# CESNET/GPUJPEG

Hardware: AMD Instinct MI355X
Metric: Mpix/s encode+decode (8K RGB q75) (higher is better)
Workload: dtype f32

## Files before the change

### gpujpeg_amd/csrc/gj_enc_assemble.hip

```cpp
#include "gj_enc_internal.h"

#define GJ_GATHER_PRELOAD 8
#define GJ_GATHER_MARK_DW 2048
__global__ __launch_bounds__(256) void k_gather(const GjTail T0)
{
    GjTail T = T0;
    {
        const size_t fz = blockIdx.z;
        T.piece += fz * T0.f_tail; T.group += fz * T0.f_tail; T.group_other += fz * T0.f_tail;
        T.temp += fz * T0.f_temp; T.seg_bytes += fz * T0.f_seg; T.seg_ff += fz * T0.f_seg;
        T.jpeg += fz * T0.f_jpeg; T.d_result += fz * 2;
        if (T.h_result) T.h_result += fz * 2;
    }
    __shared__ uint32_t s_tmp[4];
    __shared__ __attribute__((aligned(16))) uint8_t s_mark[4][GJ_GATHER_MARK_DW];
    const int i = threadIdx.x, lane = i & 63, wave = i >> 6;
    const uint32_t P = T.npieces, NG = T.ngroups;
    const uint32_t p0 = blockIdx.x * 4u, p = p0 + (uint32_t)wave;
    const bool have = p < P;
    if (blockIdx.x == 0)
        for (uint32_t g = i; g < NG; g += 256) T.group_other[g] = 0;
    const uint32_t scan = gj_tail_scan_of(T, have ? p : 0u);
    const uint32_t t = (have ? p : 0u) - gj_pick4(T.scan_first, scan), seg0 = t * T.spt, scan_segs = gj_pick4(T.segs, scan);
    const uint32_t nseg = have ? min(T.spt, scan_segs - seg0) : 0u;
    const uint32_t s0 = gj_pick4(T.seg_first, scan) + seg0;
    const uint64_t src_block = (uint64_t)gj_pick4(T.block_first, scan) + (uint64_t)seg0 * T.seg_blocks;
    const uint32_t* const src = reinterpret_cast<const uint32_t*>(T.temp + src_block * GJ_TEMP_BYTES_PER_BLOCK);
    const uint64_t room = T.temp_blocks > src_block ? T.temp_blocks - src_block : 0u;
    const uint32_t src_dw = (uint32_t)min((uint64_t)nseg * T.seg_blocks, room) * (GJ_TEMP_BYTES_PER_BLOCK / 4u);
    const uint32_t ga = p0 >> 5;
    uint32_t before = 0, all = 0;
    for (uint32_t g0 = 0; g0 < NG; g0 += 1024) {
        uint32_t v[4];
#pragma unroll
        for (int u = 0; u < 4; u++) {
            const uint32_t g = g0 + (uint32_t)u * 256u + (uint32_t)i;
            v[u] = g < NG ? T.group[g] : 0u;
        }
#pragma unroll
        for (int u = 0; u < 4; u++) {
            const uint32_t g = g0 + (uint32_t)u * 256u + (uint32_t)i;
            all += v[u];
            before += g < ga ? v[u] : 0u;
        }
    }
    if ((uint32_t)i < (p0 & 31u)) before += T.piece[(ga << 5) + i];
    uint32_t in_front = 0;
    if (wave > 0 && have) in_front += T.piece[p0];
    if (wave > 1 && have) in_front += T.piece[p0 + 1];
    if (wave > 2 && have) in_front += T.piece[p0 + 2];
    uint32_t nb = 0, ff = 0;
    if ((uint32_t)lane < nseg) {
        nb = T.seg_bytes[s0 + lane];
        ff = T.seg_ff[s0 + lane];
    }
    uint32_t pre[GJ_GATHER_PRELOAD];
#pragma unroll
    for (int m = 0; m < GJ_GATHER_PRELOAD; m++) {
        const uint32_t d = (uint32_t)m * 64u + (uint32_t)lane;
        pre[m] = d < src_dw ? src[d] : 0u;
    }
    uint32_t done_bytes, all_bytes;
    gj_wg256_incl_scan(before, s_tmp, &done_bytes);
    gj_wg256_incl_scan(all, s_tmp, &all_bytes);
    const uint64_t total = (uint64_t)T.main_hdr + gj_pick4(T.hdr_end, gj_tail_scan_of(T, P - 1)) + all_bytes + 2u;
    const bool overflow = total > T.capacity;
    if (p0 + 4 >= P && i == 0) {
        T.d_result[0] = (uint32_t)total;
        T.d_result[1] = overflow ? 1u : 0u;
        if (T.h_result) {
            T.h_result[0] = (uint32_t)total;
            T.h_result[1] = overflow ? 1u : 0u;
        }
    }
    if (!have || overflow) return;
    const uint32_t F = T.main_hdr + gj_pick4(T.hdr_end, scan) + done_bytes + in_front;
    uint8_t* const out = T.jpeg;
    if (t == 0) {
        const uint32_t h1 = gj_pick4(T.hdr_end, scan), h0 = scan == 0 ? 0u : gj_pick4(T.hdr_end, scan - 1);
        for (uint32_t b = lane; b < h1 - h0; b += 64) out[F - (h1 - h0) + b] = T.scan_hdr[h0 + b];
    }
    const uint32_t last = scan_segs - seg0 - 1u;
    const uint32_t ndw = (nb + 3u) >> 2, olen = nb + ff + ((uint32_t)lane < nseg && (uint32_t)lane != last ? 2u : 0u);
    const uint32_t dwi = gj_wave_incl_scan(ndw), dwb = dwi - ndw;
    const uint32_t oi = gj_wave_incl_scan(olen), ob = F + oi - olen;
    const uint32_t ffi = gj_wave_incl_scan(ff);
    const uint32_t total_dw = (uint32_t)__builtin_amdgcn_readlane((int)dwi, 63);
    const uint32_t end = F + (uint32_t)__builtin_amdgcn_readlane((int)oi, 63);
    if (p == P - 1 && lane == 0) {
        out[end] = 0xFF;
        out[end + 1] = 0xD9;
    }
    const uint32_t seg_a = ob - 4u * dwb - (ffi - ff);
    const uint32_t seg_e = (dwi - 1u) | ((nb - 4u * (ndw - 1u)) << 28);
    uint8_t* const mark = s_mark[wave];
    uint32_t ffrun = 0, segs_before = 0;
    for (uint32_t c0 = 0; c0 < total_dw; c0 += GJ_GATHER_MARK_DW) {
        const uint32_t c1 = min(total_dw, c0 + (uint32_t)GJ_GATHER_MARK_DW);
        gj_wave_sync();
#pragma unroll
        for (int z = 0; z < GJ_GATHER_MARK_DW / 256; z++) reinterpret_cast<uint32_t*>(mark)[z * 64 + lane] = 0;
        gj_wave_sync();
        if ((uint32_t)lane < nseg && dwb >= c0 && dwb < c1) mark[dwb - c0] = 1;
        gj_wave_sync();
        for (uint32_t m = c0 >> 6; m * 64u < c1; m++) {
            const uint32_t d = m * 64u + (uint32_t)lane;
            const bool live = d < total_dw;
            uint32_t v = 0;
            if (m < GJ_GATHER_PRELOAD) {
#pragma unroll
                for (int q = 0; q < GJ_GATHER_PRELOAD; q++)
                    if (m == (uint32_t)q) v = pre[q];
            } else if (live) {
                v = src[d];
            }
            const uint32_t seg = gj_wave_incl_scan(live ? mark[d - c0] : 0u) + segs_before - 1u;
            const int sidx = (int)((live ? seg : 0u) << 2);
            const uint32_t a = (uint32_t)__builtin_amdgcn_ds_bpermute(sidx, (int)seg_a), e = (uint32_t)__builtin_amdgcn_ds_bpermute(sidx, (int)seg_e);
            const bool ends = live && d == (e & 0x0FFFFFFFu);
            const int vb = live ? (ends ? (int)(e >> 28) : 4) : 0;
            const uint32_t ffm = live ? ((v & 0x7F7F7F7Fu) + 0x01010101u) & v & 0x80808080u : 0u;
            const uint32_t ffc = (uint32_t)__builtin_popcount(ffm);
            const uint32_t fi = gj_wave_incl_scan(ffc) + ffrun;
            if (live) {
                uint32_t q = a + 4u * d + (fi - ffc);
                if (ffc == 0 && vb == 4) {
                    *reinterpret_cast<gj_u32_unaligned*>(out + q) = v;
                    q += 4;
                } else {
#pragma unroll
                    for (int b = 0; b < 4; b++)
                        if (b < vb) {
                            const uint32_t byte = (v >> (8 * b)) & 0xFFu;
                            out[q++] = (uint8_t)byte;
                            if (byte == 0xFFu) out[q++] = 0;
                        }
                }
                if (ends && seg != last) {
                    out[q] = 0xFF;
                    out[q + 1] = (uint8_t)(0xD0 + ((seg0 + seg) & 7u));
                }
            }
            ffrun = (uint32_t)__builtin_amdgcn_readlane((int)fi, 63);
            segs_before = (uint32_t)__builtin_amdgcn_readlane((int)seg, 63) + 1u;
        }
    }
}

__device__ __forceinline__ uint32_t gj_segment_out_size(const gj_enc_job& J, int s, uint32_t* hdr)
{
    const GjSeg sg = gj_segment(J.g, s);
    *hdr = 0;
    if (sg.first_in_scan) {
        const int scan = J.g.interleaved ? 0 : sg.comp;
        *hdr = J.scan_hdr_offset[scan + 1] - J.scan_hdr_offset[scan];
    }
    return J.d_seg_bytes[s] + J.d_seg_ff[s] + (sg.last_in_scan ? 0u : 2u);
}

__device__ __forceinline__ uint32_t gj_wg1024_incl_scan(uint32_t v, uint32_t* s_w, uint32_t* total)
{
    const int lane = threadIdx.x & 63, wave = threadIdx.x >> 6;
    const uint32_t inc = gj_wave_incl_scan(v);
    __syncthreads();
    if (lane == 63) s_w[wave] = inc;
    __syncthreads();
    uint32_t off = 0, all = 0;
#pragma unroll
    for (int w = 0; w < 16; w++) {
        const uint32_t x = s_w[w];
        if (w < wave) off += x;
        all += x;
    }
    if (total) *total = all;
    return inc + off;
}

__global__ __launch_bounds__(1024) void k_scan_segments(const gj_enc_job J, unsigned long long* __restrict__ partial, const uint32_t epoch)
{
    __shared__ uint32_t s_w[16];
    const int S = J.g.segment_count;
    const int s = blockIdx.x * 1024 + threadIdx.x;
    uint32_t hdr = 0, v = 0;
    if (s < S) v = gj_segment_out_size(J, s, &hdr);
    uint32_t total;
    const uint32_t inc = gj_wg1024_incl_scan(v + hdr, s_w, &total);
    if (threadIdx.x == 0)
        __hip_atomic_store(&partial[blockIdx.x], ((unsigned long long)epoch << 32) | total, __ATOMIC_RELEASE, __HIP_MEMORY_SCOPE_AGENT);
    uint32_t pre = 0;
    for (unsigned t = threadIdx.x; t < blockIdx.x; t += 1024) {
        unsigned long long p;
        do {
            p = __hip_atomic_load(&partial[t], __ATOMIC_ACQUIRE, __HIP_MEMORY_SCOPE_AGENT);
        } while ((uint32_t)(p >> 32) != epoch);
        pre += (uint32_t)p;
    }
    uint32_t base;
    gj_wg1024_incl_scan(pre, s_w, &base);
    base += J.main_hdr_size;
    if (s < S) J.d_seg_out[s] = base + inc - v;
    if (s == S - 1) {
        const uint32_t end = base + inc;
        const uint32_t size = end + 2;
        J.d_seg_out[S] = end;
        J.d_result[0] = size;
        J.d_result[1] = (uint64_t)size > J.jpeg_capacity ? 1u : 0u;
        if (J.h_result) {
            J.h_result[0] = size;
            J.h_result[1] = (uint64_t)size > J.jpeg_capacity ? 1u : 0u;
        }
    }
}

__global__ __launch_bounds__(256) void k_assemble(const gj_enc_job J)
{
    const gj_geom& g = J.g;
    const int s0 = (blockIdx.x * 4 + (threadIdx.x >> 6)) * GJ_ASM_SEGS;
    const int lane = threadIdx.x & 63;
    if (s0 >= g.segment_count || J.d_result[1]) return;
    uint8_t* out = J.d_jpeg;
    uint32_t raw4[GJ_ASM_SEGS], o4[GJ_ASM_SEGS], w4[GJ_ASM_SEGS];
    const uint8_t* src4[GJ_ASM_SEGS];
#pragma unroll
    for (int q = 0; q < GJ_ASM_SEGS; q++) {
        const int s = min(s0 + q, g.segment_count - 1);
        raw4[q] = s0 + q < g.segment_count ? J.d_seg_bytes[s] : 0u;
        o4[q] = J.d_seg_out[s];
        src4[q] = J.d_temp + gj_segment(g, s).first_block * GJ_TEMP_BYTES_PER_BLOCK;
    }
#pragma unroll
    for (int q = 0; q < GJ_ASM_SEGS; q++) w4[q] = (uint32_t)lane * 4u < raw4[q] ? *reinterpret_cast<const uint32_t*>(src4[q] + lane * 4) : 0u;
#pragma unroll
    for (int q = 0; q < GJ_ASM_SEGS; q++) {
        const int s = s0 + q;
        if (s >= g.segment_count) break;
        const GjSeg sg = gj_segment(g, s);
        const uint32_t raw = raw4[q];
        const uint8_t* src = src4[q];
        uint32_t o = o4[q];
        if (sg.first_in_scan) {
            const int scan = g.interleaved ? 0 : sg.comp;
            const uint32_t h0 = J.scan_hdr_offset[scan], hn = J.scan_hdr_offset[scan + 1] - h0;
            for (uint32_t b = lane; b < hn; b += 64) out[o - hn + b] = J.d_scan_hdr[h0 + b];
        }
        for (uint32_t c0 = 0; c0 < raw; c0 += 256) {
            const uint32_t idx = c0 + lane * 4;
            uint32_t w = w4[q];
            int vb = 0;
            if (idx < raw) {
                if (c0) w = *reinterpret_cast<const uint32_t*>(src + idx);
                vb = (int)min(4u, raw - idx);
            }
            int cnt = vb;
#pragma unroll
            for (int b = 0; b < 4; b++)
                if (b < vb && ((w >> (8 * b)) & 0xFFu) == 0xFFu) cnt++;
            const uint32_t inc = gj_wave_incl_scan((uint32_t)cnt);
            uint32_t p = o + inc - (uint32_t)cnt;
#pragma unroll
            for (int b = 0; b < 4; b++) {
                if (b < vb) {
                    const uint32_t byte = (w >> (8 * b)) & 0xFFu;
                    out[p++] = (uint8_t)byte;
                    if (byte == 0xFFu) out[p++] = 0;
                }
            }
            o += (uint32_t)__builtin_amdgcn_readlane((int)inc, 63);
        }
        if (lane == 0) {
            if (!sg.last_in_scan) {
                out[o] = 0xFF;
                out[o + 1] = (uint8_t)(0xD0 + (sg.index_in_scan & 7));
            }
            if (s == g.segment_count - 1) {
                out[o] = 0xFF;
                out[o + 1] = 0xD9;
            }
        }
    }
}

#define GJ_MAX_HEADER_SIZE (65536 - 100)
__global__ __launch_bounds__(256) void k_segment_info(const gj_enc_job J)
{
    const gj_geom& g = J.g;
    const int s = blockIdx.x * 256 + threadIdx.x;
    if (s >= g.segment_count || J.d_result[1]) return;
    const GjSeg sg = gj_segment(g, s);
    const int scan = g.interleaved ? 0 : sg.comp;
    const int first = g.interleaved ? 0 : g.comp[scan].first_segment;
    const int segs = g.interleaved ? g.segment_count : g.comp[scan].segment_count;
    const uint32_t data0 = J.d_seg_out[first];
    const uint32_t hdr_begin = data0 - (J.scan_hdr_offset[scan + 1] - J.scan_hdr_offset[scan]);
    for (int e = sg.index_in_scan; e <= (sg.last_in_scan ? segs : sg.index_in_scan); e++) {
        uint32_t pos;
        if (e < segs) pos = J.d_seg_out[first + e] - data0;
        else pos = J.d_seg_out[first + segs - 1] + J.d_seg_bytes[first + segs - 1] + J.d_seg_ff[first + segs - 1] - data0;
        const uint32_t byte = (uint32_t)e * 4u;
        const uint32_t chunk = byte / GJ_MAX_HEADER_SIZE, within = byte % GJ_MAX_HEADER_SIZE;
        uint8_t* p = J.d_jpeg + hdr_begin + J.scan_info_payload[scan] + chunk * (GJ_MAX_HEADER_SIZE + 5u) + within;
        p[0] = (uint8_t)(pos >> 24); p[1] = (uint8_t)(pos >> 16); p[2] = (uint8_t)(pos >> 8); p[3] = (uint8_t)pos;
    }
}
```

### gpujpeg_amd/csrc/gj_encode.hip

```cpp
#include "gj_enc_internal.h"

static GjTail gj_make_tail(const gj_enc_job* job, const unsigned pieces, const unsigned (&scan_first)[GJ_MAX_COMP], const unsigned spt)
{
    const gj_geom& g = job->g;
    GjTail T;
    for (int s = 0; s < GJ_MAX_COMP; s++) {
        T.scan_first[s] = scan_first[s];
        T.hdr_end[s] = job->scan_hdr_offset[s + 1];
        const bool own_scan = !g.interleaved && s < g.comp_count;
        T.seg_first[s] = own_scan ? (uint32_t)g.comp[s].first_segment : 0u;
        T.segs[s] = own_scan ? (uint32_t)g.comp[s].segment_count : (uint32_t)g.segment_count;
        T.block_first[s] = own_scan ? (uint32_t)(g.comp[s].data_offset / 64) : 0u;
    }
    T.spt = spt;
    T.seg_blocks = (uint32_t)g.seg_blocks;
    const unsigned ngcap = GJ_TAIL_GROUPS_CAP(g.segment_count);
    T.group = job->d_tail + (job->tail_set & 1) * ngcap;
    T.group_other = job->d_tail + ((job->tail_set + 1) & 1) * ngcap;
    T.ngroups = (pieces + 31) / 32;
    T.piece = job->d_tail + 2 * ngcap;
    T.npieces = pieces;
    T.temp = job->d_temp;
    T.temp_blocks = (uint64_t)g.block_count;
    T.seg_bytes = job->d_seg_bytes;
    T.seg_ff = job->d_seg_ff;
    T.jpeg = job->d_jpeg;
    T.capacity = job->jpeg_capacity;
    T.scan_hdr = job->d_scan_hdr;
    T.main_hdr = job->main_hdr_size;
    T.d_result = job->d_result;
    T.h_result = job->h_result;
    const bool batch = job->batch.count > 1;
    T.f_raw = batch ? job->batch.raw : 0;
    T.f_temp = batch ? job->batch.temp : 0;
    T.f_jpeg = batch ? job->batch.jpeg : 0;
    T.f_seg = batch ? job->batch.seg : 0;
    T.f_tail = batch ? job->batch.tail : 0;
    return T;
}


static int gj_blocks_kernel_mode(const gj_geom& g)
{
    if (g.no_transform) return 1;
    if (g.pixel_format != GJ_PF_444_P012 || g.comp_count != 3) return -1;
    const int from = g.color_space, to = g.color_space_internal;
    const bool none = from == to || from == GJ_CS_NONE || to == GJ_CS_NONE;
    if (!none && !(from == GJ_CS_RGB && (to == GJ_CS_BT601 || to == GJ_CS_BT601_256 || to == GJ_CS_BT709))) return -1;
    return 0;
}

static bool gj_is_uyvy_layout(const gj_enc_job* job)
{
    const gj_geom& g = job->g;
    return job->use_fused && g.pixel_format == GJ_PF_422_P1020 && g.comp_count == 3 && g.no_transform == 0 &&
           (g.color_space == g.color_space_internal || g.color_space == GJ_CS_NONE || g.color_space_internal == GJ_CS_NONE) &&
           g.comp[0].samp_h == 2 && g.comp[0].samp_v == 1 && g.comp[1].samp_h == 1 && g.comp[1].samp_v == 1 && g.comp[2].samp_h == 1 &&
           g.comp[2].samp_v == 1 && g.comp[0].blocks_x == 2 * g.comp[1].blocks_x && g.comp[0].blocks_y == g.comp[1].blocks_y &&
           g.comp[2].blocks_x == g.comp[1].blocks_x && g.comp[2].blocks_y == g.comp[1].blocks_y;
}
static int gj_tile_kernel(const gj_enc_job* job)
{
    const gj_geom& g = job->g;
    if (job->stage != GJ_ENC_STAGE_ALL) return 0;
    const bool segs_ok = g.restart_interval > 0 && g.seg_blocks <= 256 && g.seg_blocks >= 256 / GJ_ENC_MAX_SPT;
    gj_encode_kernel_t whole = (job->use_fused && !job->keep_coefs) ? gj_encode_kernel(g) : nullptr;
    if (whole && job->tune.enc_by_blocks > 0 && gj_blocks_kernel_mode(g) == 0) whole = nullptr;
    if (gj_is_uyvy_layout(job) && !job->keep_coefs && g.interleaved && segs_ok && g.blocks_per_mcu == 4 && g.mcu_count == g.comp[1].blocks_x * g.comp[1].blocks_y &&
        g.comp[1].type == g.comp[2].type && !job->tune.enc_no_whole422)
        return 1;
    if (!whole && job->use_fused && !job->keep_coefs && segs_ok && gj_blocks_kernel_mode(g) >= 0) return 2;
    return whole ? 3 : 0;
}

extern "C" int gj_hip_encode_batchable(const gj_enc_job* job)
{
    return job->use_fused && !job->keep_coefs && !job->channel_remap && !job->flipped && !job->segment_info && gj_tile_kernel(job) != 0;
}

extern "C" int gj_hip_encode_tiles(const gj_enc_job* job) { return gj_tile_kernel(job) != 0; }

extern "C" int gj_hip_encode(const gj_enc_job* job, gj_stream_t stream, gj_event_t ev[GJ_ENC_EVENTS])
{
    hipStream_t st = (hipStream_t)stream;
    const gj_geom& g = job->g;
    if (g.blocks_per_mcu > GJ_MAX_MCU_BLOCKS) return -1;
    const unsigned frames = job->batch.count > 1 ? job->batch.count : 1u;
    if (frames > 1 && (!gj_hip_encode_batchable(job) || frames > 65535u)) return -1;
    if (job->stage != GJ_ENC_STAGE_ALL && (frames > 1 || (job->stage == GJ_ENC_STAGE_COUNT && !job->d_huff_freq))) return -1;
    gj_hip_note_reset();
    const bool code_only = job->stage == GJ_ENC_STAGE_CODE;
    if (ev && !code_only) GJ_HIP_CHECK(hipEventRecord((hipEvent_t)ev[0], st));
    if (job->channel_remap && !code_only) {
        const unsigned n = (unsigned)g.width * (unsigned)g.height;
        hipLaunchKernelGGL(k_channel_remap, dim3((n + 255) / 256), dim3(256), 0, st, g, const_cast<uint8_t*>(job->d_raw), job->channel_remap & 0xFFFFu);
    }
    bool tiles = true;
    GjTail T;
    T.npieces = 0;
    const int tile_kernel = gj_tile_kernel(job);
    gj_encode_kernel_t whole = tile_kernel == 3 ? gj_encode_kernel(g) : nullptr;
    gj_fused_kernel_t fused = job->use_fused ? gj_fused_kernel(g) : nullptr;
    const bool uyvy = gj_is_uyvy_layout(job);
    if (tile_kernel == 1) {
        if (ev) GJ_HIP_CHECK(hipEventRecord((hipEvent_t)ev[1], st));
        if (ev) GJ_HIP_CHECK(hipEventRecord((hipEvent_t)ev[2], st));
        const int spt = 256 / g.seg_blocks;
        const unsigned wgs = ((unsigned)g.segment_count + spt - 1) / spt;
        T = gj_make_tail(job, wgs, {0u, ~0u, ~0u, ~0u}, (unsigned)spt);
        hipLaunchKernelGGL(gj_encode_uyvy422_kernel(), dim3(wgs, 1, frames), dim3(256), 0, st, g, job->d_raw, job->d_fwd_q[0], job->d_fwd_q[1], job->d_huff_lut,
                           job->d_temp, job->d_seg_bytes, job->d_seg_ff, T);
    } else if (tile_kernel == 2) {
        if (ev) GJ_HIP_CHECK(hipEventRecord((hipEvent_t)ev[1], st));
        if (ev) GJ_HIP_CHECK(hipEventRecord((hipEvent_t)ev[2], st));
        const int spt = 256 / g.seg_blocks;
        unsigned wgs = 0, scan_first[GJ_MAX_COMP] = {0u, ~0u, ~0u, ~0u};
        if (g.interleaved) wgs = ((unsigned)g.segment_count + spt - 1) / spt;
        else
            for (int c = 0; c < g.comp_count; c++) {
                scan_first[c] = wgs;
                wgs += ((unsigned)g.comp[c].segment_count + spt - 1) / spt;
            }
        T = gj_make_tail(job, wgs, scan_first, (unsigned)spt);
        hipLaunchKernelGGL(gj_encode_blocks_kernel(gj_blocks_kernel_mode(g) != 0), dim3(wgs, 1, frames), dim3(256), 0, st, g, job->d_raw, job->d_fwd_q[0],
                           job->d_fwd_q[1], job->d_huff_lut, job->d_temp, job->d_seg_bytes, job->d_seg_ff, T);
    } else if (whole) {
        if (ev) GJ_HIP_CHECK(hipEventRecord((hipEvent_t)ev[1], st));
        if (ev) GJ_HIP_CHECK(hipEventRecord((hipEvent_t)ev[2], st));
        const int spt = 256 / g.seg_blocks;
        const unsigned wgs = ((unsigned)g.comp[0].segment_count + spt - 1) / spt;
        T = gj_make_tail(job, 3 * wgs, {0u, wgs, 2 * wgs, ~0u}, (unsigned)spt);
        const unsigned split_up_to = job->tune.enc_split >= 0 ? (unsigned)job->tune.enc_split : (unsigned)gj_hip_cu_count() * 4u / 3u;
        const bool split = wgs * frames <= split_up_to;
        if (split) whole = gj_encode_kernel(g, true);
        unsigned grid_x = wgs;
        const unsigned tail = job->tune.enc_tail >= 0 ? (unsigned)job->tune.enc_tail : 32u;
        T.tail_from = 0xFFFFFFFFu;
        T.tiles = wgs;
        if (!split && frames == 1 && tail > 0 && wgs > tail && (job->tune.enc_tail > 0 || wgs > (unsigned)gj_hip_cu_count() * 4u)) {
            T.tail_from = wgs - tail;
            grid_x = wgs + 2u * tail;
        }
        hipLaunchKernelGGL(whole, dim3(grid_x, split ? 3 : 1, frames), dim3(256), 0, st, g, job->d_raw, job->d_fwd_q[0], job->d_fwd_q[1], job->d_huff_lut, job->d_temp,
                           job->d_seg_bytes, job->d_seg_ff, T);
    } else {
    tiles = false;
    if (code_only) {
    } else if (uyvy) {
        if (ev) GJ_HIP_CHECK(hipEventRecord((hipEvent_t)ev[1], st));
        const unsigned nm = (unsigned)(g.comp[1].blocks_x * g.comp[1].blocks_y);
        hipLaunchKernelGGL(gj_fused_uyvy422_kernel(), dim3((nm + 255) / 256), dim3(256), 0, st, g, job->d_raw, job->d_coefs, job->d_fwd_q[0], job->d_fwd_q[1]);
    } else if (fused) {
        if (ev) GJ_HIP_CHECK(hipEventRecord((hipEvent_t)ev[1], st));
        const unsigned nb = (unsigned)(g.comp[0].blocks_x * g.comp[0].blocks_y);
        hipLaunchKernelGGL(fused, dim3((nb + 255) / 256), dim3(256), 0, st, g, job->d_raw, job->d_coefs, job->d_fwd_q[0],
                           job->d_fwd_q[1]);
    } else {
        if (g.no_transform) {
            hipLaunchKernelGGL(k_copy_planes_in, dim3(2048), dim3(256), 0, st, g, job->d_raw, job->d_planes);
        } else {
            const unsigned n = (unsigned)g.raw_width * (unsigned)g.height;
            hipLaunchKernelGGL(k_preprocess, dim3((n + 255) / 256), dim3(256), 0, st, g, job->d_raw, job->d_planes);
        }
        if (job->flipped) hipLaunchKernelGGL(k_flip_planes, dim3(1024), dim3(256), 0, st, g, job->d_planes);
        if (ev) GJ_HIP_CHECK(hipEventRecord((hipEvent_t)ev[1], st));
        hipLaunchKernelGGL(k_dct, dim3(((unsigned)g.block_count + 255) / 256), dim3(256), 0, st, g, job->d_planes, job->d_coefs,
                           job->d_fwd_q[0], job->d_fwd_q[1]);
    }
    if (job->stage == GJ_ENC_STAGE_COUNT) {
        if (ev) GJ_HIP_CHECK(hipEventRecord((hipEvent_t)ev[6], st));
        GJ_HIP_CHECK(hipMemsetAsync(job->d_huff_freq, 0, 1024 * sizeof(uint32_t), st));
        const unsigned total = (unsigned)g.segment_count * (unsigned)g.seg_blocks;
        const unsigned fill = (unsigned)gj_hip_cu_count() * 4u, wgs = (total + 255) / 256 < fill ? (total + 255) / 256 : fill;
        hipLaunchKernelGGL(k_huffman_count, dim3(wgs), dim3(256), 0, st, g, job->d_coefs, job->d_huff_freq);
        if (ev) GJ_HIP_CHECK(hipEventRecord((hipEvent_t)ev[7], st));
        return (hipGetLastError() == hipSuccess && !gj_hip_noted()) ? 0 : -1;
    }
    if (ev) GJ_HIP_CHECK(hipEventRecord((hipEvent_t)ev[2], st));
    const int B = g.seg_blocks;
    const int spt = B <= 256 ? 256 / B : 1;
    const unsigned tiles = ((unsigned)g.segment_count + spt - 1) / spt;
    hipLaunchKernelGGL(k_huffman, dim3(tiles), dim3(256), 0, st, g, job->d_coefs, job->d_huff_lut, job->d_temp, job->d_seg_bytes,
                       job->d_seg_ff);
    }
    if (ev) GJ_HIP_CHECK(hipEventRecord((hipEvent_t)ev[3], st));
    if (tiles)
        hipLaunchKernelGGL(k_gather, dim3((T.npieces + 3) / 4, 1, frames), dim3(256), 0, st, T);
    const bool seg_info = job->segment_info && g.restart_interval > 0;
    const unsigned scan_wgs = ((unsigned)g.segment_count + 1023) / 1024;
    if (!tiles || seg_info)
        hipLaunchKernelGGL(k_scan_segments, dim3(scan_wgs), dim3(1024), 0, st, *job, (unsigned long long*)job->d_scan_partial, job->epoch);
    if (ev) GJ_HIP_CHECK(hipEventRecord((hipEvent_t)ev[4], st));
    if (!tiles)
        hipLaunchKernelGGL(k_assemble, dim3(((unsigned)g.segment_count + 4 * GJ_ASM_SEGS - 1) / (4 * GJ_ASM_SEGS)), dim3(256), 0, st, *job);
    if (seg_info)
        hipLaunchKernelGGL(k_segment_info, dim3(((unsigned)g.segment_count + 255) / 256), dim3(256), 0, st, *job);
    if (ev) GJ_HIP_CHECK(hipEventRecord((hipEvent_t)ev[5], st));
    return (hipGetLastError() == hipSuccess && !gj_hip_noted()) ? 0 : -1;
}
```

Measured before the change: 179,200.

## Vectorize gather to four dwords per lane and use wave-local prefix sums

The gather kernel now has each lane process four consecutive dwords through uint4 loads. Segment indices come from a packed 4-byte mark word, FF counts are summed per lane before one wave scan, and the common no-FF, non-ending dwords take a fast store path. The workgroup-wide scans over group sums are replaced by per-wave scans, so each wave reads all groups itself and no LDS barrier is needed. This cuts scan and bpermute overhead per byte moved, but adds redundant per-wave group reads and assumes 16-byte alignment of the source.

```diff
diff --git a/gpujpeg_amd/csrc/gj_enc_assemble.hip b/gpujpeg_amd/csrc/gj_enc_assemble.hip
--- a/gpujpeg_amd/csrc/gj_enc_assemble.hip
+++ b/gpujpeg_amd/csrc/gj_enc_assemble.hip
@@ -1,6 +1,6 @@
 #include "gj_enc_internal.h"
 
-#define GJ_GATHER_PRELOAD 8
+#define GJ_GATHER_PRELOAD 2
 #define GJ_GATHER_MARK_DW 2048
 __global__ __launch_bounds__(256) void k_gather(const GjTail T0)
 {
@@ -12,7 +12,6 @@
         T.jpeg += fz * T0.f_jpeg; T.d_result += fz * 2;
         if (T.h_result) T.h_result += fz * 2;
     }
-    __shared__ uint32_t s_tmp[4];
     __shared__ __attribute__((aligned(16))) uint8_t s_mark[4][GJ_GATHER_MARK_DW];
     const int i = threadIdx.x, lane = i & 63, wave = i >> 6;
     const uint32_t P = T.npieces, NG = T.ngroups;
@@ -30,21 +29,21 @@
     const uint32_t src_dw = (uint32_t)min((uint64_t)nseg * T.seg_blocks, room) * (GJ_TEMP_BYTES_PER_BLOCK / 4u);
     const uint32_t ga = p0 >> 5;
     uint32_t before = 0, all = 0;
-    for (uint32_t g0 = 0; g0 < NG; g0 += 1024) {
+    for (uint32_t g0 = 0; g0 < NG; g0 += 256) {
         uint32_t v[4];
 #pragma unroll
         for (int u = 0; u < 4; u++) {
-            const uint32_t g = g0 + (uint32_t)u * 256u + (uint32_t)i;
+            const uint32_t g = g0 + (uint32_t)u * 64u + (uint32_t)lane;
             v[u] = g < NG ? T.group[g] : 0u;
         }
 #pragma unroll
         for (int u = 0; u < 4; u++) {
-            const uint32_t g = g0 + (uint32_t)u * 256u + (uint32_t)i;
+            const uint32_t g = g0 + (uint32_t)u * 64u + (uint32_t)lane;
             all += v[u];
             before += g < ga ? v[u] : 0u;
         }
     }
-    if ((uint32_t)i < (p0 & 31u)) before += T.piece[(ga << 5) + i];
+    if ((uint32_t)lane < (p0 & 31u)) before += T.piece[(ga << 5) + lane];
     uint32_t in_front = 0;
     if (wave > 0 && have) in_front += T.piece[p0];
     if (wave > 1 && have) in_front += T.piece[p0 + 1];
@@ -54,15 +53,14 @@
         nb = T.seg_bytes[s0 + lane];
         ff = T.seg_ff[s0 + lane];
     }
-    uint32_t pre[GJ_GATHER_PRELOAD];
+    uint4 pre[GJ_GATHER_PRELOAD];
 #pragma unroll
     for (int m = 0; m < GJ_GATHER_PRELOAD; m++) {
-        const uint32_t d = (uint32_t)m * 64u + (uint32_t)lane;
-        pre[m] = d < src_dw ? src[d] : 0u;
-    }
-    uint32_t done_bytes, all_bytes;
-    gj_wg256_incl_scan(before, s_tmp, &done_bytes);
-    gj_wg256_incl_scan(all, s_tmp, &all_bytes);
+        const uint32_t d = (uint32_t)m * 256u + (uint32_t)lane * 4u;
+        pre[m] = d < src_dw ? *reinterpret_cast<const uint4*>(src + d) : make_uint4(0, 0, 0, 0);
+    }
+    const uint32_t done_bytes = (uint32_t)__builtin_amdgcn_readlane((int)gj_wave_incl_scan(before), 63);
+    const uint32_t all_bytes = (uint32_t)__builtin_amdgcn_readlane((int)gj_wave_incl_scan(all), 63);
     const uint64_t total = (uint64_t)T.main_hdr + gj_pick4(T.hdr_end, gj_tail_scan_of(T, P - 1)) + all_bytes + 2u;
     const bool overflow = total > T.capacity;
     if (p0 + 4 >= P && i == 0) {
@@ -103,46 +101,79 @@
         gj_wave_sync();
         if ((uint32_t)lane < nseg && dwb >= c0 && dwb < c1) mark[dwb - c0] = 1;
         gj_wave_sync();
-        for (uint32_t m = c0 >> 6; m * 64u < c1; m++) {
-            const uint32_t d = m * 64u + (uint32_t)lane;
-            const bool live = d < total_dw;
-            uint32_t v = 0;
+        for (uint32_t m = c0 >> 8; m * 256u < c1; m++) {
+            const uint32_t d0 = m * 256u + (uint32_t)lane * 4u;
+            uint4 ld = make_uint4(0, 0, 0, 0);
             if (m < GJ_GATHER_PRELOAD) {
 #pragma unroll
                 for (int q = 0; q < GJ_GATHER_PRELOAD; q++)
-                    if (m == (uint32_t)q) v = pre[q];
-            } else if (live) {
-                v = src[d];
-            }
-            const uint32_t seg = gj_wave_incl_scan(live ? mark[d - c0] : 0u) + segs_before - 1u;
-            const int sidx = (int)((live ? seg : 0u) << 2);
-            const uint32_t a = (uint32_t)__builtin_amdgcn_ds_bpermute(sidx, (int)seg_a), e = (uint32_t)__builtin_amdgcn_ds_bpermute(sidx, (int)seg_e);
-            const bool ends = live && d == (e & 0x0FFFFFFFu);
-            const int vb = live ? (ends ? (int)(e >> 28) : 4) : 0;
-            const uint32_t ffm = live ? ((v & 0x7F7F7F7Fu) + 0x01010101u) & v & 0x80808080u : 0u;
-            const uint32_t ffc = (uint32_t)__builtin_popcount(ffm);
-            const uint32_t fi = gj_wave_incl_scan(ffc) + ffrun;
-            if (live) {
-                uint32_t q = a + 4u * d + (fi - ffc);
-                if (ffc == 0 && vb == 4) {
-                    *reinterpret_cast<gj_u32_unaligned*>(out + q) = v;
-                    q += 4;
-                } else {
-#pragma unroll
-                    for (int b = 0; b < 4; b++)
-                        if (b < vb) {
-                            const uint32_t byte = (v >> (8 * b)) & 0xFFu;
-                            out[q++] = (uint8_t)byte;
-                            if (byte == 0xFFu) out[q++] = 0;
-                        }
+                    if (m == (uint32_t)q) ld = pre[q];
+            } else if (d0 < min(total_dw, src_dw)) {
+                ld = *reinterpret_cast<const uint4*>(src + d0);
+            }
+            uint32_t v[4] = {ld.x, ld.y, ld.z, ld.w}, seg[4], a[4], e[4], ffm[4], ffc[4];
+            uint32_t lm = 0xFu;
+            if (m * 256u + 256u > total_dw) {
+                lm = d0 < total_dw ? 0xFu >> (4u - min(4u, total_dw - d0)) : 0u;
+#pragma unroll
+                for (int j = 0; j < 4; j++) v[j] = (lm >> j) & 1u ? v[j] : 0u;
+            }
+            const uint32_t mk = *reinterpret_cast<const uint32_t*>(mark + (d0 - c0));
+            const uint32_t starts = gj_wave_incl_scan((uint32_t)__builtin_popcount(mk)) + segs_before;
+            seg[3] = starts - 1u;
+            seg[2] = seg[3] - (mk >> 24);
+            seg[1] = seg[2] - ((mk >> 16) & 1u);
+            seg[0] = seg[1] - ((mk >> 8) & 1u);
+#pragma unroll
+            for (int j = 0; j < 4; j++) {
+                a[j] = (uint32_t)__builtin_amdgcn_ds_bpermute((int)(seg[j] << 2), (int)seg_a);
+                e[j] = (uint32_t)__builtin_amdgcn_ds_bpermute((int)(seg[j] << 2), (int)seg_e);
+            }
+            uint32_t ffs = 0;
+#pragma unroll
+            for (int j = 0; j < 4; j++) {
+                ffm[j] = ((v[j] & 0x7F7F7F7Fu) + 0x01010101u) & v[j] & 0x80808080u;
+                ffc[j] = (uint32_t)__builtin_popcount(ffm[j]);
+                ffs += ffc[j];
+            }
+            const uint32_t fi = gj_wave_incl_scan(ffs) + ffrun;
+            uint32_t q[4], slow = 0;
+            q[0] = 4u * d0 + (fi - ffs);
+            q[1] = q[0] + 4u + ffc[0];
+            q[2] = q[1] + 4u + ffc[1];
+            q[3] = q[2] + 4u + ffc[2];
+#pragma unroll
+            for (int j = 0; j < 4; j++) {
+                q[j] += a[j];
+                slow |= (uint32_t)((ffm[j] != 0u) | (d0 + (uint32_t)j == (e[j] & 0x0FFFFFFFu))) << j;
+            }
+            const uint32_t plain = lm & ~slow;
+#pragma unroll
+            for (int j = 0; j < 4; j++)
+                if ((plain >> j) & 1u) *reinterpret_cast<gj_u32_unaligned*>(out + q[j]) = v[j];
+            while (slow) {
+                const uint32_t j = (uint32_t)__builtin_ctz(slow);
+                slow &= slow - 1u;
+                const uint32_t vj = j == 0 ? v[0] : j == 1 ? v[1] : j == 2 ? v[2] : v[3];
+                const uint32_t ej = j == 0 ? e[0] : j == 1 ? e[1] : j == 2 ? e[2] : e[3];
+                const uint32_t sj = j == 0 ? seg[0] : j == 1 ? seg[1] : j == 2 ? seg[2] : seg[3];
+                uint32_t qj = j == 0 ? q[0] : j == 1 ? q[1] : j == 2 ? q[2] : q[3];
+                const bool ends = d0 + j == (ej & 0x0FFFFFFFu);
+                const int vb = ends ? (int)(ej >> 28) : 4;
+#pragma unroll
+                for (int b = 0; b < 4; b++)
+                    if (b < vb) {
+                        const uint32_t byte = (vj >> (8 * b)) & 0xFFu;
+                        out[qj++] = (uint8_t)byte;
+                        if (byte == 0xFFu) out[qj++] = 0;
+                    }
+                if (ends && sj != last) {
+                    out[qj] = 0xFF;
+                    out[qj + 1] = (uint8_t)(0xD0 + ((seg0 + sj) & 7u));
                 }
-                if (ends && seg != last) {
-                    out[q] = 0xFF;
-                    out[q + 1] = (uint8_t)(0xD0 + ((seg0 + seg) & 7u));
-                }
             }
             ffrun = (uint32_t)__builtin_amdgcn_readlane((int)fi, 63);
-            segs_before = (uint32_t)__builtin_amdgcn_readlane((int)seg, 63) + 1u;
+            segs_before = (uint32_t)__builtin_amdgcn_readlane((int)starts, 63);
         }
     }
 }
```

New measurement: 180,300 (median of 6 runs). About the same (+0.6%).

## Restructure gather kernel with per-wave scans, 16-byte loads and marker-byte segment ends

Applied to the files above, without the earlier changes.

The gather kernel now lets each wave compute its own prefix over piece/group sizes instead of doing workgroup-wide scans through shared memory. It drops the per-segment FF-count input and stops using bpermute lookups. Instead, segment ends are encoded as marker bytes in LDS, holding padding and restart info, and output positions are derived from one running scan per 16-byte chunk. Source data is loaded and stored in uint4 chunks, with a divergent slow path only for dwords that contain 0xFF bytes or segment ends. The change adds a host-side alignment check on the temp buffer, plus optional trace hooks. In exchange it risks more lane-serialised slow-path work whenever chunks hold 0xFF bytes.

```diff
diff --git a/gpujpeg_amd/csrc/gj_enc_assemble.hip b/gpujpeg_amd/csrc/gj_enc_assemble.hip
--- a/gpujpeg_amd/csrc/gj_enc_assemble.hip
+++ b/gpujpeg_amd/csrc/gj_enc_assemble.hip
@@ -1,150 +1,182 @@
 #include "gj_enc_internal.h"
 
-#define GJ_GATHER_PRELOAD 8
+#define GJ_GATHER_PRELOAD 2
 #define GJ_GATHER_MARK_DW 2048
+#ifndef GJ_GATHER_STORE16
+#define GJ_GATHER_STORE16 1
+#endif
+#ifdef GJ_TRACE_PHASES
+static __device__ int gj_trace_stop_g = 1 << 30;
+extern "C" GJ_HIP_API int gj_hip_trace_stop_gather(int n) { return hipMemcpyToSymbol(HIP_SYMBOL(gj_trace_stop_g), &n, sizeof n) == hipSuccess ? 0 : -1; }
+#define GJ_TRACE_G(slot) do { if ((slot) >= gj_trace_stop_g) __builtin_amdgcn_endpgm(); } while (0)
+#else
+#define GJ_TRACE_G(slot) ((void)0)
+#endif
+#define GJ_GATHER_PAD 0x07070707u
+#define GJ_GATHER_RST 0x18181818u
 __global__ __launch_bounds__(256) void k_gather(const GjTail T0)
 {
     GjTail T = T0;
     {
         const size_t fz = blockIdx.z;
         T.piece += fz * T0.f_tail; T.group += fz * T0.f_tail; T.group_other += fz * T0.f_tail;
-        T.temp += fz * T0.f_temp; T.seg_bytes += fz * T0.f_seg; T.seg_ff += fz * T0.f_seg;
+        T.temp += fz * T0.f_temp; T.seg_bytes += fz * T0.f_seg;
         T.jpeg += fz * T0.f_jpeg; T.d_result += fz * 2;
         if (T.h_result) T.h_result += fz * 2;
     }
-    __shared__ uint32_t s_tmp[4];
     __shared__ __attribute__((aligned(16))) uint8_t s_mark[4][GJ_GATHER_MARK_DW];
-    const int i = threadIdx.x, lane = i & 63, wave = i >> 6;
+    const uint32_t lane = threadIdx.x & 63u;
+    const uint32_t wave = (uint32_t)__builtin_amdgcn_readfirstlane((int)(threadIdx.x >> 6));
     const uint32_t P = T.npieces, NG = T.ngroups;
-    const uint32_t p0 = blockIdx.x * 4u, p = p0 + (uint32_t)wave;
-    const bool have = p < P;
+    const uint32_t p = blockIdx.x * 4u + wave;
     if (blockIdx.x == 0)
-        for (uint32_t g = i; g < NG; g += 256) T.group_other[g] = 0;
-    const uint32_t scan = gj_tail_scan_of(T, have ? p : 0u);
-    const uint32_t t = (have ? p : 0u) - gj_pick4(T.scan_first, scan), seg0 = t * T.spt, scan_segs = gj_pick4(T.segs, scan);
-    const uint32_t nseg = have ? min(T.spt, scan_segs - seg0) : 0u;
+        for (uint32_t g = threadIdx.x; g < NG; g += 256) T.group_other[g] = 0;
+    if (p >= P) return;
+    const uint32_t scan = gj_tail_scan_of(T, p);
+    const uint32_t t = p - gj_pick4(T.scan_first, scan), seg0 = t * T.spt, scan_segs = gj_pick4(T.segs, scan);
+    const uint32_t nseg = min(T.spt, scan_segs - seg0);
     const uint32_t s0 = gj_pick4(T.seg_first, scan) + seg0;
     const uint64_t src_block = (uint64_t)gj_pick4(T.block_first, scan) + (uint64_t)seg0 * T.seg_blocks;
     const uint32_t* const src = reinterpret_cast<const uint32_t*>(T.temp + src_block * GJ_TEMP_BYTES_PER_BLOCK);
     const uint64_t room = T.temp_blocks > src_block ? T.temp_blocks - src_block : 0u;
     const uint32_t src_dw = (uint32_t)min((uint64_t)nseg * T.seg_blocks, room) * (GJ_TEMP_BYTES_PER_BLOCK / 4u);
-    const uint32_t ga = p0 >> 5;
+    const uint32_t ga = p >> 5;
     uint32_t before = 0, all = 0;
-    for (uint32_t g0 = 0; g0 < NG; g0 += 1024) {
+    for (uint32_t g0 = 0; g0 < NG; g0 += 256) {
         uint32_t v[4];
 #pragma unroll
         for (int u = 0; u < 4; u++) {
-            const uint32_t g = g0 + (uint32_t)u * 256u + (uint32_t)i;
+            const uint32_t g = g0 + (uint32_t)u * 64u + lane;
             v[u] = g < NG ? T.group[g] : 0u;
         }
 #pragma unroll
         for (int u = 0; u < 4; u++) {
-            const uint32_t g = g0 + (uint32_t)u * 256u + (uint32_t)i;
+            const uint32_t g = g0 + (uint32_t)u * 64u + lane;
             all += v[u];
             before += g < ga ? v[u] : 0u;
         }
     }
-    if ((uint32_t)i < (p0 & 31u)) before += T.piece[(ga << 5) + i];
-    uint32_t in_front = 0;
-    if (wave > 0 && have) in_front += T.piece[p0];
-    if (wave > 1 && have) in_front += T.piece[p0 + 1];
-    if (wave > 2 && have) in_front += T.piece[p0 + 2];
-    uint32_t nb = 0, ff = 0;
-    if ((uint32_t)lane < nseg) {
-        nb = T.seg_bytes[s0 + lane];
-        ff = T.seg_ff[s0 + lane];
-    }
-    uint32_t pre[GJ_GATHER_PRELOAD];
+    if (lane < (p & 31u)) before += T.piece[(ga << 5) + lane];
+    const uint32_t nb = lane < nseg ? T.seg_bytes[s0 + lane] : 0u;
+    uint4 pre[GJ_GATHER_PRELOAD];
 #pragma unroll
     for (int m = 0; m < GJ_GATHER_PRELOAD; m++) {
-        const uint32_t d = (uint32_t)m * 64u + (uint32_t)lane;
-        pre[m] = d < src_dw ? src[d] : 0u;
-    }
-    uint32_t done_bytes, all_bytes;
-    gj_wg256_incl_scan(before, s_tmp, &done_bytes);
-    gj_wg256_incl_scan(all, s_tmp, &all_bytes);
+        const uint32_t d = (uint32_t)m * 256u + 4u * lane;
+        pre[m] = d < src_dw ? *reinterpret_cast<const uint4*>(src + d) : make_uint4(0u, 0u, 0u, 0u);
+    }
+    const uint32_t done_bytes = (uint32_t)__builtin_amdgcn_readlane((int)gj_wave_incl_scan(before), 63);
+    const uint32_t all_bytes = (uint32_t)__builtin_amdgcn_readlane((int)gj_wave_incl_scan(all), 63);
     const uint64_t total = (uint64_t)T.main_hdr + gj_pick4(T.hdr_end, gj_tail_scan_of(T, P - 1)) + all_bytes + 2u;
     const bool overflow = total > T.capacity;
-    if (p0 + 4 >= P && i == 0) {
+    uint8_t* const out = T.jpeg;
+    if (p == P - 1 && lane == 0) {
         T.d_result[0] = (uint32_t)total;
         T.d_result[1] = overflow ? 1u : 0u;
         if (T.h_result) {
             T.h_result[0] = (uint32_t)total;
             T.h_result[1] = overflow ? 1u : 0u;
         }
-    }
-    if (!have || overflow) return;
-    const uint32_t F = T.main_hdr + gj_pick4(T.hdr_end, scan) + done_bytes + in_front;
-    uint8_t* const out = T.jpeg;
+        if (!overflow) {
+            out[(uint32_t)total - 2u] = 0xFF;
+            out[(uint32_t)total - 1u] = 0xD9;
+        }
+    }
+    if (overflow) return;
+    const uint32_t F = T.main_hdr + gj_pick4(T.hdr_end, scan) + done_bytes;
     if (t == 0) {
         const uint32_t h1 = gj_pick4(T.hdr_end, scan), h0 = scan == 0 ? 0u : gj_pick4(T.hdr_end, scan - 1);
         for (uint32_t b = lane; b < h1 - h0; b += 64) out[F - (h1 - h0) + b] = T.scan_hdr[h0 + b];
     }
+    GJ_TRACE_G(1);
     const uint32_t last = scan_segs - seg0 - 1u;
-    const uint32_t ndw = (nb + 3u) >> 2, olen = nb + ff + ((uint32_t)lane < nseg && (uint32_t)lane != last ? 2u : 0u);
-    const uint32_t dwi = gj_wave_incl_scan(ndw), dwb = dwi - ndw;
-    const uint32_t oi = gj_wave_incl_scan(olen), ob = F + oi - olen;
-    const uint32_t ffi = gj_wave_incl_scan(ff);
+    const uint32_t ndw = (nb + 3u) >> 2;
+    const uint32_t dwi = gj_wave_incl_scan(ndw);
     const uint32_t total_dw = (uint32_t)__builtin_amdgcn_readlane((int)dwi, 63);
-    const uint32_t end = F + (uint32_t)__builtin_amdgcn_readlane((int)oi, 63);
-    if (p == P - 1 && lane == 0) {
-        out[end] = 0xFF;
-        out[end + 1] = 0xD9;
-    }
-    const uint32_t seg_a = ob - 4u * dwb - (ffi - ff);
-    const uint32_t seg_e = (dwi - 1u) | ((nb - 4u * (ndw - 1u)) << 28);
+    const uint32_t note = ((1u << (4u * ndw - nb)) - 1u) | (lane != last ? 0x18u | (((seg0 + lane) & 7u) << 5) : 0u);
+    GJ_TRACE_G(2);
     uint8_t* const mark = s_mark[wave];
-    uint32_t ffrun = 0, segs_before = 0;
+    uint32_t pos = F;
     for (uint32_t c0 = 0; c0 < total_dw; c0 += GJ_GATHER_MARK_DW) {
         const uint32_t c1 = min(total_dw, c0 + (uint32_t)GJ_GATHER_MARK_DW);
         gj_wave_sync();
-#pragma unroll
-        for (int z = 0; z < GJ_GATHER_MARK_DW / 256; z++) reinterpret_cast<uint32_t*>(mark)[z * 64 + lane] = 0;
+        static_assert(GJ_GATHER_MARK_DW == 2048, "two clearing stores of 1024 bytes");
+        reinterpret_cast<uint4*>(mark)[lane] = make_uint4(0u, 0u, 0u, 0u);
+        if (c1 - c0 > 1024u) reinterpret_cast<uint4*>(mark)[64u + lane] = make_uint4(0u, 0u, 0u, 0u);
         gj_wave_sync();
-        if ((uint32_t)lane < nseg && dwb >= c0 && dwb < c1) mark[dwb - c0] = 1;
+        if (lane < nseg && dwi - 1u >= c0 && dwi - 1u < c1) mark[dwi - 1u - c0] = (uint8_t)note;
         gj_wave_sync();
-        for (uint32_t m = c0 >> 6; m * 64u < c1; m++) {
-            const uint32_t d = m * 64u + (uint32_t)lane;
-            const bool live = d < total_dw;
-            uint32_t v = 0;
-            if (m < GJ_GATHER_PRELOAD) {
+        for (uint32_t r0 = c0; r0 < c1; r0 += 256u) {
+            const uint32_t d0 = r0 + 4u * lane;
+            uint4 x = make_uint4(0u, 0u, 0u, 0u);
+            if (r0 < GJ_GATHER_PRELOAD * 256u) {
 #pragma unroll
                 for (int q = 0; q < GJ_GATHER_PRELOAD; q++)
-                    if (m == (uint32_t)q) v = pre[q];
-            } else if (live) {
-                v = src[d];
-            }
-            const uint32_t seg = gj_wave_incl_scan(live ? mark[d - c0] : 0u) + segs_before - 1u;
-            const int sidx = (int)((live ? seg : 0u) << 2);
-            const uint32_t a = (uint32_t)__builtin_amdgcn_ds_bpermute(sidx, (int)seg_a), e = (uint32_t)__builtin_amdgcn_ds_bpermute(sidx, (int)seg_e);
-            const bool ends = live && d == (e & 0x0FFFFFFFu);
-            const int vb = live ? (ends ? (int)(e >> 28) : 4) : 0;
-            const uint32_t ffm = live ? ((v & 0x7F7F7F7Fu) + 0x01010101u) & v & 0x80808080u : 0u;
-            const uint32_t ffc = (uint32_t)__builtin_popcount(ffm);
-            const uint32_t fi = gj_wave_incl_scan(ffc) + ffrun;
-            if (live) {
-                uint32_t q = a + 4u * d + (fi - ffc);
-                if (ffc == 0 && vb == 4) {
-                    *reinterpret_cast<gj_u32_unaligned*>(out + q) = v;
-                    q += 4;
-                } else {
+                    if (r0 == (uint32_t)q * 256u) x = pre[q];
+            } else if (d0 < total_dw && d0 < src_dw) {
+                x = *reinterpret_cast<const uint4*>(src + d0);
+            }
+            uint32_t v[4] = {x.x, x.y, x.z, x.w};
+            const uint32_t M = *reinterpret_cast<const uint32_t*>(mark + (d0 - c0));
+            const uint32_t nlive = (uint32_t)min(4, max(0, (int)(total_dw - d0)));
+            if (r0 + 256u > total_dw) {
+#pragma unroll
+                for (int k = 1; k < 4; k++) v[k] = (uint32_t)k < nlive ? v[k] : 0u;
+                v[0] = nlive ? v[0] : 0u;
+            }
+            uint32_t ffm[4], ffc = 0;
+#pragma unroll
+            for (int k = 0; k < 4; k++) {
+                ffm[k] = ((v[k] & 0x7F7F7F7Fu) + 0x01010101u) & v[k] & 0x80808080u;
+                ffc += (uint32_t)__builtin_popcount(ffm[k]);
+            }
+            const uint32_t bytes = 4u * nlive + ffc + (uint32_t)__builtin_popcount(M & GJ_GATHER_RST) - (uint32_t)__builtin_popcount(M & GJ_GATHER_PAD);
+            const uint32_t bi = gj_wave_incl_scan(bytes);
+            uint32_t q = pos + bi - bytes;
+            pos += (uint32_t)__builtin_amdgcn_readlane((int)bi, 63);
+            uint32_t dirty = 0, qk[4];
+            if ((M | ffm[0] | ffm[1] | ffm[2] | ffm[3]) == 0 && nlive == 4) {
+#if GJ_GATHER_STORE16
+                __builtin_memcpy(out + q, v, 16);
+#else
+#pragma unroll
+                for (int k = 0; k < 4; k++) *reinterpret_cast<gj_u32_unaligned*>(out + q + 4 * k) = v[k];
+#endif
+            } else {
+#pragma unroll
+                for (int k = 0; k < 4; k++) {
+                    const uint32_t mk = (M >> (8 * k)) & 0xFFu;
+                    qk[k] = q;
+                    if ((uint32_t)k < nlive) {
+                        if ((mk | ffm[k]) == 0) *reinterpret_cast<gj_u32_unaligned*>(out + q) = v[k];
+                        else dirty |= 1u << k;
+                    }
+                    q += 4u + (uint32_t)__builtin_popcount(ffm[k]) + (uint32_t)__builtin_popcount(mk & 0x18u) - (uint32_t)__builtin_popcount(mk & 0x07u);
+                }
+            }
+            while (__ballot(dirty != 0)) {
+                if (dirty) {
+                    const uint32_t k = (uint32_t)__builtin_ctz(dirty);
+                    dirty &= dirty - 1u;
+                    const uint32_t w = k == 0 ? v[0] : k == 1 ? v[1] : k == 2 ? v[2] : v[3];
+                    uint32_t o = k == 0 ? qk[0] : k == 1 ? qk[1] : k == 2 ? qk[2] : qk[3];
+                    const uint32_t mk = (M >> (8u * k)) & 0xFFu;
+                    const int vb = 4 - __builtin_popcount(mk & 0x07u);
 #pragma unroll
                     for (int b = 0; b < 4; b++)
                         if (b < vb) {
-                            const uint32_t byte = (v >> (8 * b)) & 0xFFu;
-                            out[q++] = (uint8_t)byte;
-                            if (byte == 0xFFu) out[q++] = 0;
+                            const uint32_t byte = (w >> (8 * b)) & 0xFFu;
+                            out[o++] = (uint8_t)byte;
+                            if (byte == 0xFFu) out[o++] = 0;
                         }
+                    if (mk & 0x08u) {
+                        out[o] = 0xFF;
+                        out[o + 1] = (uint8_t)(0xD0u + (mk >> 5));
+                    }
                 }
-                if (ends && seg != last) {
-                    out[q] = 0xFF;
-                    out[q + 1] = (uint8_t)(0xD0 + ((seg0 + seg) & 7u));
-                }
-            }
-            ffrun = (uint32_t)__builtin_amdgcn_readlane((int)fi, 63);
-            segs_before = (uint32_t)__builtin_amdgcn_readlane((int)seg, 63) + 1u;
-        }
-    }
+            }
+        }
+    }
+    GJ_TRACE_G(3);
 }
 
 __device__ __forceinline__ uint32_t gj_segment_out_size(const gj_enc_job& J, int s, uint32_t* hdr)
diff --git a/gpujpeg_amd/csrc/gj_encode.hip b/gpujpeg_amd/csrc/gj_encode.hip
--- a/gpujpeg_amd/csrc/gj_encode.hip
+++ b/gpujpeg_amd/csrc/gj_encode.hip
@@ -1,4 +1,5 @@
 #include "gj_enc_internal.h"
+#include <assert.h>
 
 static GjTail gj_make_tail(const gj_enc_job* job, const unsigned pieces, const unsigned (&scan_first)[GJ_MAX_COMP], const unsigned spt)
 {
@@ -184,6 +185,11 @@
                        job->d_seg_ff);
     }
     if (ev) GJ_HIP_CHECK(hipEventRecord((hipEvent_t)ev[3], st));
+    static_assert(GJ_TEMP_BYTES_PER_BLOCK % 16 == 0, "k_gather's 16-byte loads");
+    if (tiles && ((((uintptr_t)job->d_temp) & 15u) != 0 || (frames > 1 && (job->batch.temp & 15u) != 0))) {
+        assert(!"d_temp and its batch stride are multiples of 16 bytes");
+        return -1;
+    }
     if (tiles)
         hipLaunchKernelGGL(k_gather, dim3((T.npieces + 3) / 4, 1, frames), dim3(256), 0, st, T);
     const bool seg_info = job->segment_info && g.restart_interval > 0;
```

Measured after the change: 179,700 before, 182,100 after (median of 6 runs). +1.3%, better.
